# Nathan494326/Husky-Rover-MPPI-IsaacSim

Measured on AMD Instinct MI355X. Metric: MPPI steps/sec at K=65536 H=100 on 750x750 costmap; 1/2/4/8-GPU scaling, higher is better.
Workload: dtype f32

## Files before the change

### husky-rover-mppi-isaacsim_amd/csrc/mppi_kernels.hip

```cpp
#include <hip/hip_runtime.h>

#include <algorithm>
#include <type_traits>
#include <stdint.h>

#include "mppi_detmath.h"
#include "mppi_kernels.h"

namespace mppi {

constexpr bool kFastMath = false;
constexpr bool kChainFast = true;

struct Recip {
  float b, y;
};
__device__ __forceinline__ bool div_ok(float v) {
  const float a = fabsf(v);
  return a >= 9.094947017729282e-13f && a <= 1.099511627776e12f;
}
template <bool F>
__device__ __forceinline__ Recip rc(float b, bool& bad) {
  Recip r;
  r.b = b;
// ... 511 lines not shown
  if (p.mode == 2) return b;
  if (j == 0) return (double)p.m;
  return (double)p.ea * a + (double)p.eb * b;
}
__device__ __forceinline__ PairScale ld_scale(const PairScale* ps) { return *ps; }
__device__ __forceinline__ double pair_apply_raw(const PairScale p, double a, double b, int j) {
  double r = (double)p.ea * a + (double)p.eb * b;
  asm volatile("" : "+v"(r));
  const double n = j == 0 ? (double)p.m : r;
  return p.mode == 1 ? a : (p.mode == 2 ? b : n);
}
__device__ __forceinline__ double pair_apply_sel(const PairScale& ps, double a, double b, int j) {
  return pair_apply_raw(ps, a, b, j);
}

template <int G>
__device__ __forceinline__ void group_scales(const float (&m)[G], float T, PairScale (&ps)[G - 1]) {
  float cur[G];
#pragma unroll
  for (int i = 0; i < G; ++i) cur[i] = m[i];
  int base = 0;
#pragma unroll
  for (int w = G / 2; w >= 1; w >>= 1) {
#pragma unroll
    for (int i = 0; i < w; ++i) {
      ps[base + i] = pair_scale(cur[2 * i], cur[2 * i + 1], T);
      cur[i] = ps[base + i].m;
    }
    base += w;
  }
}
template <int G>
__device__ __forceinline__ double group_apply(const PairScale* ps, const double (&v)[G], int j) {
  double cur[G];
#pragma unroll
  for (int i = 0; i < G; ++i) cur[i] = v[i];
  int base = 0;
#pragma unroll
  for (int w = G / 2; w >= 1; w >>= 1) {
#pragma unroll
    for (int i = 0; i < w; ++i) cur[i] = pair_apply(ps[base + i], cur[2 * i], cur[2 * i + 1], j);
    base += w;
  }
  return cur[0];
}

template <bool FRESH, int NT = 1024>
__device__ __forceinline__ int thread_id() {
  int t = threadIdx.x;
  if constexpr (FRESH) asm volatile("" : "+v"(t));
  __builtin_assume(t >= 0 && t < NT);
  return t;
}

struct NoiseVals {
  float a1, a2, b1, b2;
};
__device__ __forceinline__ NoiseVals noise_gen(uint64_t seed, uint64_t n_base, int64_t k_offset, int blk, int n, int tj) {
  const uint64_t kg = (uint64_t)(k_offset + (int64_t)blk * 256 + tj);
  NoiseVals v;
  noise_block_pk(seed, n_base + (uint64_t)n, kg, &v.a1, &v.a2, &v.b1, &v.b2);
  return v;
}
__device__ __forceinline__ void noise_store(float* __restrict__ eps, int H, int blk, int n, int tj, const NoiseVals& v) {
  const int t = 2 * n;
  float* e1 = eps + ((size_t)blk * 2 * H + t) * 256 + tj;
  float* e2 = e1 + (size_t)H * 256;
  __hip_atomic_store(e1, v.a1, __ATOMIC_RELAXED, __HIP_MEMORY_SCOPE_AGENT);
  __hip_atomic_store(e2, v.a2, __ATOMIC_RELAXED, __HIP_MEMORY_SCOPE_AGENT);
  if (t + 1 < H) {
    __hip_atomic_store(e1 + 256, v.b1, __ATOMIC_RELAXED, __HIP_MEMORY_SCOPE_AGENT);
    __hip_atomic_store(e2 + 256, v.b2, __ATOMIC_RELAXED, __HIP_MEMORY_SCOPE_AGENT);
  }
}
__device__ __forceinline__ void noise_unit(uint64_t seed, uint64_t n_base, int64_t k_offset, int H, int blk, int n,
                                           float* __restrict__ eps, int tj) {
  noise_store(eps, H, blk, n, tj, noise_gen(seed, n_base, k_offset, blk, n, tj));
}
__device__ __forceinline__ void noise_rows(uint64_t seed, uint64_t n_base, int64_t k_offset, int H, int end,
                                           float* __restrict__ eps, int g0, int gstride, int tj) {
  const int NB = (H + 1) >> 1;
  if (g0 >= end) return;
  int blk = g0 / NB, n = g0 - blk * NB;
  const int sq = gstride / NB, sr = gstride - sq * NB;
  for (int g = g0; g < end; g += gstride) {
    noise_unit(seed, n_base, k_offset, H, blk, n, eps, tj);
    blk += sq;
    n += sr;
    if (n >= NB) {
      n -= NB;
      ++blk;
    }
  }
}
struct NoisePos {
  int q, g, blk, n;
};
__device__ __forceinline__ void noise_pos_step(NoisePos& p, int stride, int NB) {
  p.q += stride;
  p.n += (p.q >> 2) - p.g;
  p.g = p.q >> 2;
  while (p.n >= NB) {
    p.n -= NB;
    ++p.blk;
  }
}
// ... 680 lines not shown
      if constexpr (MODE == 0) {
        const int tn = min(p + 2, H - 1);
        e1r = eps_row[(size_t)tn * TB];
        e2r = eps_row[(size_t)(H + tn) * TB];
      }
    };
    using T_ = std::true_type;
    using F_ = std::false_type;
    int p = 0;
    for (const int p1 = min(H, PAIR_LAG) & ~1; p < p1; p += 2) {
      half(F_{}, T_{}, F_{}, p, eA1, eA2, cmA, cmB);
      half(T_{}, T_{}, F_{}, p + 1, eB1, eB2, cmB, cmA);
    }
    if (p == PAIR_LAG) {
      for (; p + 1 < H; p += 2) {
        half(F_{}, T_{}, T_{}, p, eA1, eA2, cmA, cmB);
        half(T_{}, T_{}, T_{}, p + 1, eB1, eB2, cmB, cmA);
      }
    }
    for (; p < H + PAIR_LAG; p += 2) {
      half(F_{}, F_{}, F_{}, p, eA1, eA2, cmA, cmB);
      if (p + 1 < H + PAIR_LAG) half(T_{}, F_{}, F_{}, p + 1, eB1, eB2, cmB, cmA);
    }
    const float cm_last = ((H - 1) & 1) ? cmB : cmA;
    if (cm_last > a.thr) ob = ob + a.pen;
    ob = ob + cm_last;
    float pf;
    if (a.pf_far) {
      const float dx = last_x - a.igx, dy = last_y - a.igy;
      pf = (dx * dx + dy * dy) * a.pf_scale;
    } else {
      pf = pf_sum;
    }
    float cost = a.w_path * pf;
    cost = cost + a.w_slope * sw;
    cost = cost + a.w_speed * sp;
    cost = cost + a.w_obs * ob;
    if (valid) a.cost_out[kl] = cost;
    cost_lds[tj] = valid ? cost : INFINITY;
  }
  __syncthreads();
  if constexpr (MODE == 0)
    leaf_records<TB, NT, true>(a, cost_lds, scratch, a.eps + (size_t)blockIdx.x * (2 * H) * TB, unom_lds, ucache,
                               a.ucache_steps);
  else
    leaf_records<TB, NT>(a, cost_lds, scratch, a.ustore + (size_t)blockIdx.x * (2 * H) * TB);
}

constexpr int kProdPrio = 1, kSidePrio = 0;
constexpr int kProdPrefetch = 2;
constexpr int ROLE_CHAIN = 0, ROLE_PROD = 1, ROLE_WHEEL = 2, ROLE_COST = 3, NROLES = 4;

template <int TB, int PROJ, int MODE, bool DUMP, bool FUSED>
__device__ __forceinline__ int roles_body(const RolloutArgs& a, int blk, unsigned* rec_cnt, int* ticket_lds = nullptr) {
  extern __shared__ __attribute__((aligned(16))) unsigned char smem_raw[];
  constexpr int NT = NROLES * TB;
  constexpr int NG = TB / 64;
  constexpr int D = PAIR_D;
  constexpr int DO = ROLES_RING_OUT;
  constexpr int RI = 4;
  static_assert(TB == 256, "UCACHE_ROW assumes 256 trajectories per workgroup");
  float* ring_in = reinterpret_cast<float*>(smem_raw);
  float* ring_out = ring_in + D * RI * TB;
  float* cost_lds = ring_out + DO * 4 * TB;
  float* sw_lds = cost_lds + TB;
  int* flags = reinterpret_cast<int*>(sw_lds + TB);
  float* unom_lds = reinterpret_cast<float*>(flags + 4 * NG);
  unsigned char* scratch = reinterpret_cast<unsigned char*>(unom_lds + ((2 * a.H + 3) & ~3));
  float* ucache = reinterpret_cast<float*>(
      smem_raw + ((size_t)(scratch - smem_raw) + ((TB + TB / 64) * 4 + 15) / 16 * 16 +
                  (size_t)(TB / 256) * (2 * a.H + 2) * sizeof(double) + 15) / 16 * 16);
  const int tid = thread_id<FUSED, NT>();
  const int wave = __builtin_amdgcn_readfirstlane(tid >> 6);
  const int role = wave / NG;
  const int grp = wave - role * NG;
  const int tj = grp * 64 + (tid & 63);
  if (a.wave_prio) {
    if (role == ROLE_CHAIN) __builtin_amdgcn_s_setprio(3);
    else if (role == ROLE_PROD) __builtin_amdgcn_s_setprio(kProdPrio);
    else __builtin_amdgcn_s_setprio(kSidePrio);
  }
  int* f_prod = flags + grp;
  int* f_chain = flags + NG + grp;
  int* f_wheel = flags + 2 * NG + grp;
  int* f_cost = flags + 3 * NG + grp;
  const int64_t kl = (int64_t)blk * TB + tj;
  const bool valid = kl < a.K;
  const int H = a.H;
  Dem dem;
  dem.init(a.Z, a.rows, a.grid, a.x_min, a.y_min, a.res, a.rinv_res, a.cdiv_res);
  dem.N = a.ntab;
  const float res_half_neg = (-a.res) / 2.0f;
  const float res_sq = a.res * a.res;
  bool nobad = false;
  const bool clk_wg = a.clk != nullptr && blockIdx.x == 0 && tid == 0;
  if (clk_wg) a.clk[4] = __builtin_amdgcn_s_memrealtime();
  const bool clk_any = a.clk != nullptr && tid == 0 && blockIdx.x < kClkBlocks;
  if (clk_any) a.clk[kClkBase + 2 * blockIdx.x] = __builtin_amdgcn_s_memrealtime();
  if (tid < 4 * NG) flags[tid] = 0;
  if constexpr (MODE == 0)
    for (int i = tid; i < 2 * H; i += NT)
      unom_lds[i] = __hip_atomic_load(i < H ? a.u_nom1 + i : a.u_nom2 + (i - H), __ATOMIC_RELAXED,
                                      __HIP_MEMORY_SCOPE_AGENT);
  __syncthreads();

  auto wait_ge = [&](const int* f, int target, int& seen) __attribute__((always_inline)) {
    if (seen >= target) return;
    int v;
    while ((v = lds_load_acquire(f)) < target) __builtin_amdgcn_s_sleep(1);
    seen = v;
  };
  using T_ = std::true_type;
  using F_ = std::false_type;
  float c_pf = 0.f, c_ob = 0.f;

  if (role == ROLE_CHAIN) {
    Traj s;
    s.x = a.x0;
    s.y = a.y0;
    {
      float q[4];
      dem.template corners<false>(s.x, s.y, q, nobad);
      const float vx = res_half_neg * (((q[1] - q[0]) - q[2]) + q[3]);
      const float vy = res_half_neg * (((q[2] - q[0]) - q[1]) + q[3]);
      const float nn = sqrtf((vx * vx + vy * vy) + res_sq * res_sq);
      const float nx = vx / nn, ny = vy / nn, nz = res_sq / nn;
      if constexpr (PROJ == 3) {
        const float d = (a.h0x * nx + a.h0y * ny) + a.h0z * nz;
        const float tx = a.h0x - d * nx, ty = a.h0y - d * ny, tz = a.h0z - d * nz;
        const float tn = sqrtf((tx * tx + ty * ty) + tz * tz);
        s.hx = tx / tn;
        s.hy = ty / tn;
        s.hz = tz / tn;
      } else {
        s.hx = a.h0x;
        s.hy = a.h0y;
        s.hz = a.h0z;
      }
    }
    int seen_prod = 0, seen_wheel = 0, seen_cost = 0;
    if constexpr (PROJ == 3) {
      const int* cons[2] = {f_wheel, f_cost};
      int seen_cons[2] = {0, 0};
      chain_wave_3d<TB, 2, DUMP, DO, !FUSED>(a, dem, s, tj, valid, kl, ring_in, ring_out, f_prod, f_chain, cons,
                                             seen_prod, seen_cons);
    } else
    for (int sc = 0; sc < H; ++sc) {
      wait_ge(f_prod, sc + 1, seen_prod);
      wait_ge(f_wheel, sc - DO + 1, seen_wheel);
      wait_ge(f_cost, sc - DO + 1, seen_cost);
      const float* ri = ring_in + (sc % D) * RI * TB + tj;
      const float v = ri[0], sn = ri[TB], cs = ri[2 * TB];
      const float cx = 0.f, cy = 0.f;
      StepOut o;
      step2d<false>(dem, a.dt, v, sn, cs, s, o, nobad);
      const float z = o.z;
      float* ro = ring_out + (sc % DO) * 4 * TB + tj;
      ro[0] = s.x;
      ro[TB] = s.y;
      ro[2 * TB] = cx;
      ro[3 * TB] = cy;
      if constexpr (DUMP) {
        if (valid) {
          const size_t o3 = ((size_t)kl * H + sc) * 3;
          if (a.d_traj) { a.d_traj[o3] = s.x; a.d_traj[o3 + 1] = s.y; a.d_traj[o3 + 2] = z; }
          if (a.d_hv) { a.d_hv[o3] = s.hx; a.d_hv[o3 + 1] = s.hy; a.d_hv[o3 + 2] = s.hz; }
        }
      }
      lds_store_release(f_chain, sc + 1);
    }
  }
  else if (role == ROLE_PROD) {
    const float* eps_row = (MODE == 0) ? a.eps + (size_t)blk * (2 * H) * TB + tj : nullptr;
    float* ust = a.ustore + (size_t)blk * (2 * H) * TB + tj;
    float L = a.wl, R = a.wr;
    float sp = 0.f;
    int seen_chain = 0;
    constexpr int PF = kProdPrefetch;
    float e[PF][2] = {};
    if constexpr (MODE == 0) {
#pragma unroll
      for (int q = 0; q < PF; ++q) {
        const int t = min(q, H - 1);
        e[q][0] = eps_row[(size_t)t * TB];
        e[q][1] = eps_row[(size_t)(H + t) * TB];
      }
    }
    auto prod = [&](int p, float& e1r, float& e2r) __attribute__((always_inline)) {
      float u1, u2;
      if constexpr (MODE == 0) {
        const int ti = min(p + 1, H - 1);
        u1 = clampf(unom_lds[ti] + a.s1 * e1r, a.min_u1, a.max_u1);
        u2 = clampf(unom_lds[H + ti] + a.s2 * e2r, a.min_u2, a.max_u2);
        if (p < a.ucache_steps) {
          ucache[(size_t)p * UCACHE_ROW + tj] = u1;
          ucache[(size_t)(a.ucache_steps + p) * UCACHE_ROW + tj] = u2;
        }
      } else {
        const size_t o = (size_t)(valid ? kl : 0) * H + p;
        u1 = a.inj_u1[o];
        u2 = a.inj_u2[o];
        ust[(size_t)p * TB] = u1;
        ust[(size_t)(H + p) * TB] = u2;
      }
      L = L * a.fa + (u1 * a.fk) * (1.0f - a.fa);
      R = R * a.fa + (u2 * a.fk) * (1.0f - a.fa);
      const float vp = clampf((L + R) / 2.0f, a.vmin, a.vmax);
      const float wp = clampf(((-L) + R) / a.rwheel, a.wmin, a.wmax);
      float sn, cs;
      if (a.small_angle) dm_sincosf_small(wp * a.dt, &sn, &cs);
      else dm_sincosf(wp * a.dt, &sn, &cs);
      const float spt = sp + (a.vmax - vp) / (vp + 0.0001f);
      sp = a.speed_on ? spt : sp;
      wait_ge(f_chain, p - D + 1, seen_chain);
      float* ri = ring_in + (p % D) * RI * TB + tj;
      ri[0] = vp;
      ri[TB] = sn;
      ri[2 * TB] = cs;
      ri[3 * TB] = 1.0f - cs;
      if constexpr (DUMP) {
        if (valid) {
          const size_t o1 = (size_t)kl * H + p;
          if (a.d_u1) a.d_u1[o1] = u1;
          if (a.d_u2) a.d_u2[o1] = u2;
          if (a.d_w) a.d_w[o1] = wp;
          if (a.d_v) a.d_v[o1] = vp;
        }
      }
      lds_store_release(f_prod, p + 1);
      if constexpr (MODE == 0) {
        const int tn = min(p + PF, H - 1);
        e1r = eps_row[(size_t)tn * TB];
        e2r = eps_row[(size_t)(H + tn) * TB];
      }
    };
    int p = 0;
    for (; p + PF <= H; p += PF) {
#pragma unroll
      for (int q = 0; q < PF; ++q) prod(p + q, e[q][0], e[q][1]);
    }
// ... 20 lines not shown
        ry = y - cy;
        rz = dem.template point<false>(rx, ry, nobad);
      }
      if constexpr (DUMP) {
        if (valid) {
          const size_t o3 = ((size_t)kl * H + sc) * 3;
          if (a.d_lw) { a.d_lw[o3] = lx; a.d_lw[o3 + 1] = ly; a.d_lw[o3 + 2] = lz; }
          if (a.d_rw) { a.d_rw[o3] = rx; a.d_rw[o3 + 1] = ry; a.d_rw[o3 + 2] = rz; }
        }
      }
    };
    auto wstep = [&](auto x_is_a, int sc) __attribute__((always_inline)) {
      constexpr bool XA = decltype(x_is_a)::value;
      float& Xlx = XA ? Alx : Blx; float& Xly = XA ? Aly : Bly; float& Xlz = XA ? Alz : Blz;
      float& Xrx = XA ? Arx : Brx; float& Xry = XA ? Ary : Bry; float& Xrz = XA ? Arz : Brz;
      const float& Ylx = XA ? Blx : Alx; const float& Yly = XA ? Bly : Aly; const float& Ylz = XA ? Blz : Alz;
      const float& Yrx = XA ? Brx : Arx; const float& Yry = XA ? Bry : Ary; const float& Yrz = XA ? Brz : Arz;
      const int i = sc - 4;
      if (i >= 0 && i < H - 3) {
        const float term = slope_term<false>(Xlx, Xly, Xlz, Ylx, Yly, Ylz, Xrx, Xry, Xrz, Yrx, Yry, Yrz, nobad);
        sw = sw + term;
      }
      contacts(sc, Xlx, Xly, Xlz, Xrx, Xry, Xrz);
      if constexpr (DUMP) {
        if (sc + 1 < H) {
          float lx, ly, lz, rx, ry, rz;
          contacts(sc + 1, lx, ly, lz, rx, ry, rz);
        }
        lds_store_release(f_wheel, min(sc + 2, H));
      } else {
        lds_store_release(f_wheel, min(sc + 2, H));
      }
    };
    int sc = 0;
    for (; sc + 2 < H; sc += 4) {
      wstep(T_{}, sc);
      wstep(F_{}, sc + 2);
    }
    if (sc < H) {
      wstep(T_{}, sc);
      sc += 2;
    }
    const int last = sc - 2;
    const int i = last - 2;
    if (i >= 0 && i < H - 3) {
      const float term = (last % 4 == 0)
          ? slope_term<false>(Blx, Bly, Blz, Alx, Aly, Alz, Brx, Bry, Brz, Arx, Ary, Arz, nobad)
          : slope_term<false>(Alx, Aly, Alz, Blx, Bly, Blz, Arx, Ary, Arz, Brx, Bry, Brz, nobad);
      sw = sw + term;
    }
    sw_lds[tj] = sw;
  } else {
    int seen_chain = 0;
    float pf_sum = 0.f, ob = 0.f, last_x = a.x0, last_y = a.y0;
    float cmA = 0.f, cmB = 0.f;
    Recip rcm;
    rcm.b = a.res_c;
    auto cstep = [&](int sc, float& cm_mine, float& cm_prev) __attribute__((always_inline)) {
      wait_ge(f_chain, sc + 1, seen_chain);
      const float* ro = ring_out + (sc % DO) * 4 * TB + tj;
      const float x = ro[0], y = ro[TB];
      cm_mine = a.cm[costmap_index<false>(a.cm_size, a.hw, rcm, x, y, nobad, a.rinv_res_c, a.cdiv_res_c)];
      const float pft = pf_sum + 10.0f * (fabsf(x - a.gx) + fabsf(y - a.gy));
      pf_sum = (sc < H - 1) ? pft : pf_sum;
      last_x = x;
      last_y = y;
      const float ob1 = (cm_prev > a.thr) ? ob + a.pen : ob;
      ob = (sc > 0) ? ob1 + cm_prev : ob;
      if constexpr (DUMP) {
      }
      lds_store_release(f_cost, sc + 1);
    };
    int sc = 0;
    for (; sc + 1 < H; sc += 2) {
      cstep(sc, cmA, cmB);
      cstep(sc + 1, cmB, cmA);
    }
    if (sc < H) cstep(sc, cmA, cmB);
    const float cm_last = ((H - 1) & 1) ? cmB : cmA;
    if (cm_last > a.thr) ob = ob + a.pen;
    ob = ob + cm_last;
    float pf;
    if (a.pf_far) {
      const float dx = last_x - a.igx, dy = last_y - a.igy;
      pf = (dx * dx + dy * dy) * a.pf_scale;
    } else {
      pf = pf_sum;
    }
    c_pf = pf;
    c_ob = ob;
  }
  __syncthreads();
  if (clk_wg) a.clk[5] = __builtin_amdgcn_s_memrealtime();
  if (role == ROLE_COST) {
    float cost = a.w_path * c_pf;
    cost = cost + a.w_slope * sw_lds[tj];
    cost = cost + a.w_speed * cost_lds[tj];
    cost = cost + a.w_obs * c_ob;
    if (valid) a.cost_out[kl] = cost;
    cost_lds[tj] = valid ? cost : INFINITY;
  }
  __syncthreads();
  if constexpr (MODE == 0)
    leaf_records<TB, NT, true, FUSED>(a, cost_lds, scratch, a.eps + (size_t)blk * (2 * H) * TB, unom_lds,
                                      ucache, a.ucache_steps, blk);
  else
// ... 637 lines not shown
    }
    v0 = v[0];
#pragma unroll
    for (int q = 0; q < 6; ++q)
      if ((1 << q) < NGW) sh[q] = ld_scale(lps + colfin_level_base(P, 4 + q) + (it_g >> (q + 1)));
  }
  int lvl = 4;
#pragma unroll
  for (int q = 0; q < 6; ++q) {
    const int k = 1 << q;
    if (k < NGW) {
      const double o = __shfl_xor(v0, k, 64);
      if (has_item && (it_g & (2 * k - 1)) == 0) v0 = pair_apply_raw(sh[q], v0, o, col);
      ++lvl;
    }
  }
  if (has_item && (it_g & (NGW - 1)) == 0) part[it_c * NG + it_g] = v0;
  __syncthreads();
  for (int stride = NGW; stride < NG; stride *= 2, ++lvl) {
    const int w = NG / (2 * stride);
    const PairScale* ps = lps + colfin_level_base(P, lvl);
    for (int it = tid; it < ncols * w; it += FIN_THREADS) {
      const int c = it % ncols, i = it / ncols;
      const int cc = (c < nc) ? c0 + c : 1;
      double* pc = part + c * NG;
      pc[2 * stride * i] = pair_apply_sel(ps[i], pc[2 * stride * i], pc[2 * stride * i + stride], cc);
    }
    __syncthreads();
  }
  if (f.mode == 0) {
    for (int c = tid; c < nc; c += FIN_THREADS) f.record_out[c0 + c] = part[c * NG];
    return true;
  }
  const double S = extra_s ? part[nc * NG] : part[(1 - c0) * NG];
  float ures = 0.0f;
  if (nblk == 1) {
    if (tid < 2 * H) ures = (S > 0.0) ? (float)(part[(tid + 2) * NG] / S) : 0.0f;
    __syncthreads();
    if (RECS_WT && tid == 0) __hip_atomic_store(rec_cnt, 0u, __ATOMIC_RELAXED, __HIP_MEMORY_SCOPE_AGENT);
  } else {
    const unsigned long long tag = (unsigned long long)f.seq << 32;
    for (int c = tid; c < nc; c += FIN_THREADS) {
      const int j = c0 + c;
      if (j >= 2) {
        const float u = (S > 0.0) ? (float)(part[c * NG] / S) : 0.0f;
        __hip_atomic_store(f.uopt + (j - 2), tag | __builtin_bit_cast(unsigned, u), __ATOMIC_RELAXED,
                           __HIP_MEMORY_SCOPE_AGENT);
      }
    }
    if (blk != nblk - 1) return true;
    int late = 0;
    if (tid < 2 * H) {
      const uint64_t t0 = __builtin_amdgcn_s_memrealtime();
      unsigned long long w = __hip_atomic_load(f.uopt + tid, __ATOMIC_RELAXED, __HIP_MEMORY_SCOPE_AGENT);
      while ((unsigned)(w >> 32) != f.seq) {
        if (__builtin_amdgcn_s_memrealtime() - t0 >= kColfinPollTicks ||
            (f.abort && __hip_atomic_load(f.abort, __ATOMIC_RELAXED, __HIP_MEMORY_SCOPE_AGENT) == f.seq)) {
          late = 1;
          break;
        }
        __builtin_amdgcn_s_sleep(1);
        w = __hip_atomic_load(f.uopt + tid, __ATOMIC_RELAXED, __HIP_MEMORY_SCOPE_AGENT);
      }
      ures = __builtin_bit_cast(float, (unsigned)w);
    }
    if (__syncthreads_or(late)) return false;
    if (RECS_WT && tid == 0) __hip_atomic_store(rec_cnt, 0u, __ATOMIC_RELAXED, __HIP_MEMORY_SCOPE_AGENT);
  }
  __syncthreads();
  finish_phase2(f, ures, smem_raw, tid, FIN_THREADS, qpre);
  return true;
}

__global__ __launch_bounds__(FIN_THREADS) void mppi_colfin_kernel(const FinishArgs f, int P, int ncol) {
  (void)colfin_body<false>(f, P, ncol, (int)blockIdx.x, (int)gridDim.x, nullptr);
}

__global__ __launch_bounds__(TAIL_THREADS) void mppi_tail_kernel(const FinishArgs f) {
  extern __shared__ __attribute__((aligned(16))) unsigned char smem_raw[];
  const int tid = threadIdx.x;
  const int H = f.H;
  float4* in4 = reinterpret_cast<float4*>(smem_raw);
  float* chain = reinterpret_cast<float*>(in4 + H + 1);
  if (tid == 0 && f.clk) f.clk[kClkServer + 8 * (f.seq & 7) + 4] = __builtin_amdgcn_s_memrealtime();
  auto ld = [&](int i) { return __hip_atomic_load(f.tail_in + i, __ATOMIC_RELAXED, __HIP_MEMORY_SCOPE_AGENT); };
  for (int t = tid; t <= H; t += TAIL_THREADS) {
    if (t == H) {
      in4[H] = make_float4(ld(0), 0.f, 0.f, 0.f);
    } else {
      const float cs = ld(2 * H + t);
      in4[t] = make_float4(ld(min(t + 1, H - 1)), ld(H + t), cs, 1.0f - cs);
    }
  }
  __syncthreads();
  Dem dem;
  dem.init(f.Z, f.rows, f.grid, f.x_min, f.y_min, f.res, f.rinv_res, f.cdiv_res);
  dem.N = f.ntab;
  optimal_rollout(f, dem, in4, chain, H, f.tail_out, tid, TAIL_THREADS);
  if (tid == 0 && f.clk) f.clk[kClkServer + 8 * (f.seq & 7) + 5] = __builtin_amdgcn_s_memrealtime();
}

__global__ __launch_bounds__(256) void mppi_bilinear_kernel(const float* __restrict__ Z, int rows,
                                                            int grid, float x_min, float y_min,
                                                            float res, const float* __restrict__ xs,
                                                            const float* __restrict__ ys,
                                                            float* __restrict__ hs, int64_t n) {
  Dem dem;
  dem.init(Z, rows, grid, x_min, y_min, res);
  const int64_t stride = (int64_t)gridDim.x * blockDim.x;
  for (int64_t i = (int64_t)blockIdx.x * blockDim.x + threadIdx.x; i < n; i += stride) {
    const float x = xs[i], y = ys[i];
    float q[4];
    bool bad = false;
    dem.template corners<true>(x, y, q, bad);
    float h = bilinear<true>(x, y, q, dem.template rr<true>(), bad);
    if (bad) {
      dem.template corners<false>(x, y, q, bad);
// ... 556 lines not shown

__global__ __launch_bounds__(256) void mppi_normal_table_kernel(const float* __restrict__ Z, int rows, int grid,
                                                                float res, float4* __restrict__ out) {
  const int64_t cols = (int64_t)grid + 1;
  const int64_t n = ((int64_t)rows + 1) * cols;
  const float res_half_neg = (-res) / 2.0f;
  const float res_sq = res * res;
  for (int64_t g = (int64_t)blockIdx.x * 256 + threadIdx.x; g < n; g += (int64_t)gridDim.x * 256) {
    const int j = (int)(g / cols) - 1, i = (int)(g % cols) - 1;
    const int r0 = clampi(j, 0, rows - 1), r1 = clampi(j + 1, 0, rows - 1);
    const int c0 = clampi(i, 0, grid - 1), c1 = clampi(i + 1, 0, grid - 1);
    const float q0 = Z[(size_t)r0 * grid + c0], q1 = Z[(size_t)r0 * grid + c1];
    const float q2 = Z[(size_t)r1 * grid + c0], q3 = Z[(size_t)r1 * grid + c1];
    bool unused = false;
    const float vx = res_half_neg * (((q1 - q0) - q2) + q3);
    const float vy = res_half_neg * (((q2 - q0) - q1) + q3);
    const Recip r = rc<false>(sq<false>((vx * vx + vy * vy) + res_sq * res_sq, unused), unused);
    out[g] = make_float4(dv<false>(vx, r, unused), dv<false>(vy, r, unused), dv<false>(res_sq, r, unused), 0.0f);
  }
}

hipError_t launch_normal_table(const float* Z, int rows, int grid, float res, float4* out, hipStream_t st) {
  const int64_t n = ((int64_t)rows + 1) * ((int64_t)grid + 1);
  const unsigned blocks = (unsigned)std::min<int64_t>((n + 255) / 256, 256 * 16);
  hipLaunchKernelGGL(mppi_normal_table_kernel, dim3(blocks), dim3(256), 0, st, Z, rows, grid, res, out);
  return hipGetLastError();
}

__global__ __launch_bounds__(256) void mppi_noise_kernel(uint64_t seed, uint64_t n_base, int64_t k_offset,
                                                         int H, int n_blocks, float* __restrict__ eps) {
  noise_rows(seed, n_base, k_offset, H, n_blocks * ((H + 1) >> 1), eps, blockIdx.x, gridDim.x, threadIdx.x);
}

struct ServerLaunch {
  RolloutArgs a;
  ServerArgs z;
};
__device__ __forceinline__ const ServerLaunch* fresh_args() {
#if __HIP_DEVICE_COMPILE__
  uint64_t v = reinterpret_cast<uint64_t>(__builtin_amdgcn_kernarg_segment_ptr());
  asm volatile("" : "+s"(v));
  return (const ServerLaunch*)reinterpret_cast<const __attribute__((address_space(4))) ServerLaunch*>(v);
#else
  return nullptr;
#endif
}

template <int TB, int PROJ>
__global__ __launch_bounds__(NROLES * TB) __attribute__((amdgpu_num_vgpr(56))) void mppi_step_server_kernel(
    const ServerLaunch args) {
  __shared__ unsigned cmd_lds[32];
  __shared__ int sh[2];
  const int tid = threadIdx.x;
  unsigned expect = args.z.first_seq;
  bool head = blockIdx.x == 0;
  for (;;) {
    const auto* L = fresh_args();
    const ServerArgs& z = L->z;
    if (tid < 64) {
      const int slot = tid < kCmdWords ? tid : 0;
      const unsigned long long* src =
          (head ? reinterpret_cast<const unsigned long long*>(z.cmd->slot) : z.relay) + slot;
      const unsigned* host_stop = reinterpret_cast<const unsigned*>(z.cmd->slot + kCmdStopSlot);
      unsigned ok = 0;
      unsigned long long w = 0;
      const uint64_t t0 = __builtin_amdgcn_s_memrealtime();
      uint64_t t_stop = t0;
      if (tid == 0 && head && z.clk) z.clk[kClkServer + 8 * (expect & 7) + 6] = t0;
      const bool forced = head && z.exit_after != 0 && expect - z.first_seq >= z.exit_after;
      while (!forced) {
        w = head ? __hip_atomic_load(src, __ATOMIC_RELAXED, __HIP_MEMORY_SCOPE_SYSTEM)
                 : __hip_atomic_load(src, __ATOMIC_RELAXED, __HIP_MEMORY_SCOPE_AGENT);
        const unsigned lo = (unsigned)w, hi = (unsigned)(w >> 32);
        const unsigned long long stop_slot = (unsigned)__builtin_amdgcn_readlane((int)lo, kCmdStopSlot);
        if (cmd_stop_hit(stop_slot, z.launch_id)) break;
        const unsigned seq0 = (unsigned)__builtin_amdgcn_readfirstlane((int)hi);
        if (__builtin_amdgcn_ballot_w64(!cmd_slot_ok(slot, w, seq0, expect)) == 0) {
          ok = 1;
          break;
        }
        const uint64_t now = __builtin_amdgcn_s_memrealtime();
        if (head) {
          if (now - t0 >= z.idle_ticks) break;
        } else {
          if (now - t_stop >= 10000) {
            t_stop = now;
            if (__hip_atomic_load(host_stop, __ATOMIC_RELAXED, __HIP_MEMORY_SCOPE_SYSTEM) == z.launch_id) break;
          }
          __builtin_amdgcn_s_sleep(2);
        }
      }
      if (ok && tid < kCmdWords) {
        if (head && tid != kCmdStopSlot)
          __hip_atomic_store(z.relay + tid, w, __ATOMIC_RELAXED, __HIP_MEMORY_SCOPE_AGENT);
        cmd_lds[tid] = (unsigned)w;
      }
      if (head && !ok && tid == 0)
        __hip_atomic_store(z.relay + kCmdStopSlot, (unsigned long long)z.launch_id, __ATOMIC_RELAXED,
                           __HIP_MEMORY_SCOPE_AGENT);
      if (tid == 0) cmd_lds[31] = ok;
      if (tid == 0 && head && z.clk && ok)
        __hip_atomic_store(z.clk + kClkServer + 8 * (cmd_lds[0] & 7), (uint64_t)__builtin_amdgcn_s_memrealtime(),
                           __ATOMIC_RELAXED, __HIP_MEMORY_SCOPE_AGENT);
    }
    __syncthreads();
    if (!cmd_lds[31]) return;
    const ServerCmd& c = *reinterpret_cast<const ServerCmd*>(cmd_lds);
    auto rd = [&](const float& x) __attribute__((always_inline)) {
      return __builtin_bit_cast(float, __builtin_amdgcn_readfirstlane(__builtin_bit_cast(int, x)));
    };
    const unsigned seq = __builtin_amdgcn_readfirstlane(c.seq);
    const int eps_slot = __builtin_amdgcn_readfirstlane(c.eps_slot);
    const int cur = __builtin_amdgcn_readfirstlane(c.cur);
    RolloutArgs a = L->a;
    a.eps = z.eps[eps_slot];
    a.u_nom1 = z.u_nom[cur];
    a.u_nom2 = z.u_nom[cur] + a.H;
    a.x0 = rd(c.x0);
    a.y0 = rd(c.y0);
    a.h0x = rd(c.h0x);
    a.h0y = rd(c.h0y);
    a.h0z = rd(c.h0z);
    a.wl = rd(c.wl);
    a.wr = rd(c.wr);
    a.gx = rd(c.gx);
    a.gy = rd(c.gy);
    a.s1 = rd(c.s1);
    a.s2 = rd(c.s2);
    a.igx = rd(c.igx);
    a.igy = rd(c.igy);
    a.pf_scale = rd(c.pf_scale);
    a.pf_far = __builtin_amdgcn_readfirstlane(c.pf_far);
    a.speed_on = __builtin_amdgcn_readfirstlane(c.speed_on);
    const int nslot = __builtin_amdgcn_readfirstlane(c.noise_slot);
    const uint64_t nbase = ((uint64_t)__builtin_amdgcn_readfirstlane(c.noise_n_base_hi) << 32) |
                           (uint32_t)__builtin_amdgcn_readfirstlane(c.noise_n_base_lo);
    const int64_t W = 4 * (int64_t)z.nroll * ((a.H + 1) >> 1);
    const int nn = z.nroll - z.fin_groups;
    const int64_t S = 2 * (int64_t)nn + z.fin_groups - 1;
    const int ticket = roles_body<TB, PROJ, 0, false, true>(a, (int)blockIdx.x, z.rec_cnt, sh);
    if (ticket == z.nroll - 1 && tid == 0 && z.clk) {
      const uint64_t now = __builtin_amdgcn_s_memrealtime();
      z.clk[kClkServer + 8 * (seq & 7) + 1] = now;
      const uint64_t t0 = __hip_atomic_load(z.clk + kClkServer + 8 * (seq & 7), __ATOMIC_RELAXED, __HIP_MEMORY_SCOPE_AGENT);
      __hip_atomic_fetch_add(z.clk + kClkSums, now - t0, __ATOMIC_RELAXED, __HIP_MEMORY_SCOPE_AGENT);
      __hip_atomic_fetch_add(z.clk + kClkSums + 1, (uint64_t)1, __ATOMIC_RELAXED, __HIP_MEMORY_SCOPE_AGENT);
    }
    const int blk = ticket - (z.nroll - z.fin_groups);
    if (blk < 0 && nslot >= 0) {
      __builtin_amdgcn_s_setprio(0);
      const int wave = __builtin_amdgcn_readfirstlane(tid >> 6);
      const int q0 = (int)(W * (2 * ticket) / S), q1 = (int)(W * (2 * ticket + 2) / S);
      noise_waves(a.seed, nbase, a.k_offset, a.H, q0 + wave, q1, NROLES * TB / 64, z.eps[nslot], tid & 63);
    }
    if (blk >= 0) {
      __builtin_amdgcn_s_setprio(0);
      if (tid == 0) {
        const uint64_t t0 = __builtin_amdgcn_s_memrealtime();
        int late = z.wait_ticks == 0;
        while (!late && ticket != z.nroll - 1 &&
               __hip_atomic_load(z.rec_cnt, __ATOMIC_RELAXED, __HIP_MEMORY_SCOPE_AGENT) < (unsigned)z.nroll) {
          if (__builtin_amdgcn_s_memrealtime() - t0 >= z.wait_ticks ||
              __hip_atomic_load(z.f.abort, __ATOMIC_RELAXED, __HIP_MEMORY_SCOPE_AGENT) == seq) {
            late = 1;
            break;
          }
          __builtin_amdgcn_s_sleep(2);
        }
        if (late) __hip_atomic_store(z.f.abort, seq, __ATOMIC_RELAXED, __HIP_MEMORY_SCOPE_AGENT);
        sh[1] = late;
      }
      __syncthreads();
      bool ok = !sh[1];
      if (ok) {
        FinishArgs f = z.f;
        const int mode = __builtin_amdgcn_readfirstlane(c.mode);
        const int slot = __builtin_amdgcn_readfirstlane(c.tail_slot);
        f.mode = mode;
        f.seq = seq;
        f.u_nom_next = z.u_nom[cur ^ 1];
        f.tail_in = z.tail_in[slot];
        f.tail_out = z.tail_out[slot];
        f.x0 = a.x0;
        f.y0 = a.y0;
        f.h0x = a.h0x;
        f.h0y = a.h0y;
        f.h0z = a.h0z;
        f.wl = a.wl;
        f.wr = a.wr;
        ok = colfin_body<true>(f, z.fin_P, z.fin_ncol, blk, z.fin_groups, z.rec_cnt);
        if (ok && blk == z.fin_groups - 1 && tid == 0 && z.clk) {
          const uint64_t now = __builtin_amdgcn_s_memrealtime();
          z.clk[kClkServer + 8 * (seq & 7) + 2] = now;
          const uint64_t t0 = __hip_atomic_load(z.clk + kClkServer + 8 * (seq & 7), __ATOMIC_RELAXED, __HIP_MEMORY_SCOPE_AGENT);
          __hip_atomic_fetch_add(z.clk + kClkSums + 2, now - t0, __ATOMIC_RELAXED, __HIP_MEMORY_SCOPE_AGENT);
          __hip_atomic_fetch_add(z.clk + kClkSums + 3, (uint64_t)1, __ATOMIC_RELAXED, __HIP_MEMORY_SCOPE_AGENT);
        }
      }
      if (!ok && tid == 0)
        __hip_atomic_store(z.f.done, seq | kDoneFail, __ATOMIC_RELAXED, __HIP_MEMORY_SCOPE_SYSTEM);
      if (nslot >= 0 && blk < z.fin_groups - 1) {
        const int wave = __builtin_amdgcn_readfirstlane(tid >> 6);
        const int q0 = (int)(W * (2 * nn + blk) / S), q1 = (int)(W * (2 * nn + blk + 1) / S);
        noise_waves(a.seed, nbase, a.k_offset, a.H, q0 + wave, q1, NROLES * TB / 64, z.eps[nslot], tid & 63);
      }
    }
    if (tid == 0) __builtin_amdgcn_fence(__ATOMIC_ACQUIRE, "agent");
    expect = seq + 1;
    head = ticket == z.nroll - 1;
    __syncthreads();
    if (tid == 0 && z.clk) {
      const uint64_t now = __builtin_amdgcn_s_memrealtime();
      if (blk < 0) __hip_atomic_fetch_max(z.clk + kClkServer + 8 * (seq & 7) + 3, now, __ATOMIC_RELAXED, __HIP_MEMORY_SCOPE_AGENT);
      __hip_atomic_fetch_max(z.clk + kClkServer + 8 * (seq & 7) + 7, now, __ATOMIC_RELAXED, __HIP_MEMORY_SCOPE_AGENT);
    }
  }
}

hipError_t launch_step_server(const RolloutArgs& a, const ServerArgs& z, size_t lds, hipStream_t st, int proj) {
  const dim3 g((unsigned)z.nroll), b(NROLES * 256);
  if (proj == 3)
    hipLaunchKernelGGL((mppi_step_server_kernel<256, 3>), g, b, lds, st, ServerLaunch{a, z});
  else
    hipLaunchKernelGGL((mppi_step_server_kernel<256, 2>), g, b, lds, st, ServerLaunch{a, z});
  return hipGetLastError();
}

hipError_t launch_noise(uint64_t seed, uint64_t n_base, int64_t k_offset, int blocks, int H, float* eps,
                        hipStream_t st, int max_groups) {
  const int NB = (H + 1) >> 1;
  const int64_t total = (int64_t)blocks * NB;
  const unsigned grid = (unsigned)std::min<int64_t>(total, std::max(max_groups, 1));
  hipLaunchKernelGGL(mppi_noise_kernel, dim3(grid), dim3(256), 0, st, seed, n_base, k_offset, H, blocks, eps);
  return hipGetLastError();
}

__global__ __launch_bounds__(256) void mppi_cdiv_verify_kernel(float b, float y, unsigned* bad) {
  const unsigned i = blockIdx.x * 256u + threadIdx.x;
  const float a = __builtin_bit_cast(float, 0x3f800000u | i);
  const float q = cdiv_f(a, b, y);
  const float ref = a / b;
  if (__builtin_bit_cast(unsigned, q) != __builtin_bit_cast(unsigned, ref)) atomicAdd(bad, 1u);
}

__global__ __launch_bounds__(64) void mppi_hold_kernel(uint64_t ticks) {
  extern __shared__ unsigned char hold_lds[];
  const uint64_t t0 = __builtin_amdgcn_s_memrealtime();
  hold_lds[threadIdx.x] = 0;
  while (__builtin_amdgcn_s_memrealtime() - t0 < ticks) __builtin_amdgcn_s_sleep(64);
}

hipError_t launch_hold(int groups, size_t lds, uint64_t ticks, hipStream_t st) {
  hipLaunchKernelGGL(mppi_hold_kernel, dim3((unsigned)groups), dim3(64), lds, st, ticks);
  return hipGetLastError();
}

hipError_t launch_cdiv_verify(float b, float y, unsigned* bad, hipStream_t st) {
  hipLaunchKernelGGL(mppi_cdiv_verify_kernel, dim3(1u << 15), dim3(256), 0, st, b, y, bad);
  return hipGetLastError();
}
// ... 21 lines not shown
```

Baseline: 13270.

## Pipeline head command polling with multiple in-flight loads and hoist first loads

Replaces the persistent server's command polling loop with a poll helper that keeps several loads in flight. The head block uses hand-written inline assembly that issues four outstanding system-scope loads, cutting latency when a new command arrives. Polling moves from wave 0 to the first cost-role wave, and leftover in-flight loads are drained after the chain role publishes its first step. The chain's first DEM corner fetch and the producer's eps prefetch are also hoisted before the role split so they overlap. The inline asm with manual vmcnt handling is fragile, and the extra outstanding loads add memory traffic.

```diff
diff --git a/husky-rover-mppi-isaacsim_amd/csrc/mppi_kernels.hip b/husky-rover-mppi-isaacsim_amd/csrc/mppi_kernels.hip
--- a/husky-rover-mppi-isaacsim_amd/csrc/mppi_kernels.hip
+++ b/husky-rover-mppi-isaacsim_amd/csrc/mppi_kernels.hip
@@ -587,6 +587,102 @@
   __builtin_assume(t >= 0 && t < NT);
   return t;
 }
+
+template <int N, typename V, typename Ld, typename Hit, typename Quit>
+__device__ __forceinline__ int poll_in_flight(V& out, Ld ld, Hit hit, Quit quit) {
+  V r[N];
+#pragma unroll
+  for (int k = 0; k < N; ++k) r[k] = ld();
+  for (;;) {
+#pragma unroll
+    for (int k = 0; k < N; ++k) {
+      const int verdict = hit(r[k]);
+      if (verdict || quit(r[k])) {
+        out = r[k];
+        return verdict;
+      }
+      r[k] = ld();
+    }
+  }
+}
+constexpr int kHeadPollDepth = 4, kFinPollDepth = 1;
+static_assert(kHeadPollDepth == 1 || kHeadPollDepth == 4, "the head's poll is written for 1 or 4 reads in flight");
+
+struct HeadSweeps {
+  unsigned long long r0 = 0, r1 = 0, r2 = 0, r3 = 0;
+  int phase = 4;
+  __device__ __forceinline__ bool resume(const unsigned long long* src, unsigned long long ref, uint64_t deadline,
+                                         unsigned long long& cand) {
+    int st;
+    uint64_t now;
+#if __HIP_DEVICE_COMPILE__
+    asm volatile(
+        "s_cmp_eq_u32 %[ph], 4\n"
+        "s_cbranch_scc0 1f\n"
+        "global_load_dwordx2 %[r0], %[src], off sc0 sc1\n"
+        "global_load_dwordx2 %[r1], %[src], off sc0 sc1\n"
+        "global_load_dwordx2 %[r2], %[src], off sc0 sc1\n"
+        "global_load_dwordx2 %[r3], %[src], off sc0 sc1\n"
+        "s_waitcnt vmcnt(3)\n"
+        "s_branch 10f\n"
+        "1:\n"
+        "s_cmp_eq_u32 %[ph], 1\n"
+        "s_cbranch_scc1 21f\n"
+        "s_cmp_eq_u32 %[ph], 2\n"
+        "s_cbranch_scc1 22f\n"
+        "s_cmp_eq_u32 %[ph], 3\n"
+        "s_cbranch_scc1 23f\n"
+#define MPPI_HEAD_SLOT(L, R, HIT)                                                    \
+        L ":\n"                                                                      \
+        "s_waitcnt vmcnt(3)\n"                                                       \
+        "v_cmp_ne_u64 vcc, " R ", %[ref]\n"                                         \
+        "s_cmp_lg_u64 vcc, 0\n"                                                      \
+        "s_cbranch_scc1 " HIT "f\n"                                                  \
+        "s_memrealtime %[now]\n"                                                     \
+        "s_waitcnt lgkmcnt(0)\n"                                                     \
+        "v_cmp_gt_u64 vcc, %[now], %[dl]\n"                                          \
+        "s_cmp_lg_u64 vcc, 0\n"                                                      \
+        "s_cbranch_scc1 90f\n"                                                       \
+        "global_load_dwordx2 " R ", %[src], off sc0 sc1\n"
+        MPPI_HEAD_SLOT("20", "%[r0]", "10")
+        MPPI_HEAD_SLOT("21", "%[r1]", "11")
+        MPPI_HEAD_SLOT("22", "%[r2]", "12")
+        MPPI_HEAD_SLOT("23", "%[r3]", "13")
+#undef MPPI_HEAD_SLOT
+        "s_branch 20b\n"
+#define MPPI_HEAD_HIT(L, R, NEXT)                                                    \
+        L ":\n"                                                                      \
+        "v_mov_b64 %[cand], " R "\n"                                                \
+        "global_load_dwordx2 " R ", %[src], off sc0 sc1\n"                          \
+        "s_mov_b32 %[ph], " NEXT "\n"                                               \
+        "s_mov_b32 %[st], 1\n"                                                       \
+        "s_branch 99f\n"
+        MPPI_HEAD_HIT("10", "%[r0]", "1")
+        MPPI_HEAD_HIT("11", "%[r1]", "2")
+        MPPI_HEAD_HIT("12", "%[r2]", "3")
+        MPPI_HEAD_HIT("13", "%[r3]", "0")
+#undef MPPI_HEAD_HIT
+        "90:\n"
+        "s_mov_b32 %[st], 0\n"
+        "99:\n"
+        : [r0] "+v"(r0), [r1] "+v"(r1), [r2] "+v"(r2), [r3] "+v"(r3), [ph] "+s"(phase), [cand] "=&v"(cand),
+          [st] "=&s"(st), [now] "=&s"(now)
+        : [src] "v"(src), [ref] "v"(ref), [dl] "v"(deadline)
+        : "vcc", "scc", "memory");
+#else
+    st = 0;
+    now = 0;
+#endif
+    (void)now;
+    return st != 0;
+  }
+  __device__ __forceinline__ void drain() {
+#if __HIP_DEVICE_COMPILE__
+    asm volatile("s_waitcnt vmcnt(0)  ; sweeps in %0 %1 %2 %3" : "+v"(r0), "+v"(r1), "+v"(r2), "+v"(r3)::"memory");
+#endif
+    phase = 4;
+  }
+};
 
 struct NoiseVals {
   float a1, a2, b1, b2;
@@ -1373,7 +1469,8 @@
 constexpr int ROLE_CHAIN = 0, ROLE_PROD = 1, ROLE_WHEEL = 2, ROLE_COST = 3, NROLES = 4;
 
 template <int TB, int PROJ, int MODE, bool DUMP, bool FUSED>
-__device__ __forceinline__ int roles_body(const RolloutArgs& a, int blk, unsigned* rec_cnt, int* ticket_lds = nullptr) {
+__device__ __forceinline__ int roles_body(const RolloutArgs& a, int blk, unsigned* rec_cnt, int* ticket_lds = nullptr,
+                                          HeadSweeps* pend = nullptr) {
   extern __shared__ __attribute__((aligned(16))) unsigned char smem_raw[];
   constexpr int NT = NROLES * TB;
   constexpr int NG = TB / 64;
@@ -1424,6 +1521,22 @@
       unom_lds[i] = __hip_atomic_load(i < H ? a.u_nom1 + i : a.u_nom2 + (i - H), __ATOMIC_RELAXED,
                                       __HIP_MEMORY_SCOPE_AGENT);
   __syncthreads();
+  constexpr int PF = kProdPrefetch;
+  const float* eps_row = (MODE == 0) ? a.eps + (size_t)blk * (2 * H) * TB + tj : nullptr;
+  float q_first[4] = {0.f, 0.f, 0.f, 0.f};
+  float e[PF][2] = {};
+  if (role == ROLE_CHAIN) {
+    dem.template corners<false>(a.x0, a.y0, q_first, nobad);
+  } else if (role == ROLE_PROD) {
+    if constexpr (MODE == 0) {
+#pragma unroll
+      for (int q = 0; q < PF; ++q) {
+        const int t = min(q, H - 1);
+        e[q][0] = eps_row[(size_t)t * TB];
+        e[q][1] = eps_row[(size_t)(H + t) * TB];
+      }
+    }
+  }
 
   auto wait_ge = [&](const int* f, int target, int& seen) __attribute__((always_inline)) {
     if (seen >= target) return;
@@ -1440,8 +1553,7 @@
     s.x = a.x0;
     s.y = a.y0;
     {
-      float q[4];
-      dem.template corners<false>(s.x, s.y, q, nobad);
+      const float (&q)[4] = q_first;
       const float vx = res_half_neg * (((q[1] - q[0]) - q[2]) + q[3]);
       const float vy = res_half_neg * (((q[2] - q[0]) - q[1]) + q[3]);
       const float nn = sqrtf((vx * vx + vy * vy) + res_sq * res_sq);
@@ -1492,21 +1604,10 @@
     }
   }
   else if (role == ROLE_PROD) {
-    const float* eps_row = (MODE == 0) ? a.eps + (size_t)blk * (2 * H) * TB + tj : nullptr;
     float* ust = a.ustore + (size_t)blk * (2 * H) * TB + tj;
     float L = a.wl, R = a.wr;
     float sp = 0.f;
     int seen_chain = 0;
-    constexpr int PF = kProdPrefetch;
-    float e[PF][2] = {};
-    if constexpr (MODE == 0) {
-#pragma unroll
-      for (int q = 0; q < PF; ++q) {
-        const int t = min(q, H - 1);
-        e[q][0] = eps_row[(size_t)t * TB];
-        e[q][1] = eps_row[(size_t)(H + t) * TB];
-      }
-    }
     auto prod = [&](int p, float& e1r, float& e2r) __attribute__((always_inline)) {
       float u1, u2;
       if constexpr (MODE == 0) {
@@ -1633,6 +1734,12 @@
     sw_lds[tj] = sw;
   } else {
     int seen_chain = 0;
+    if constexpr (FUSED) {
+      if (pend != nullptr && grp == 0) {
+        wait_ge(f_chain, 1, seen_chain);
+        pend->drain();
+      }
+    }
     float pf_sum = 0.f, ob = 0.f, last_x = a.x0, last_y = a.y0;
     float cmA = 0.f, cmB = 0.f;
     Recip rcm;
@@ -2376,17 +2483,26 @@
     int late = 0;
     if (tid < 2 * H) {
       const uint64_t t0 = __builtin_amdgcn_s_memrealtime();
-      unsigned long long w = __hip_atomic_load(f.uopt + tid, __ATOMIC_RELAXED, __HIP_MEMORY_SCOPE_AGENT);
-      while ((unsigned)(w >> 32) != f.seq) {
-        if (__builtin_amdgcn_s_memrealtime() - t0 >= kColfinPollTicks ||
-            (f.abort && __hip_atomic_load(f.abort, __ATOMIC_RELAXED, __HIP_MEMORY_SCOPE_AGENT) == f.seq)) {
-          late = 1;
-          break;
-        }
-        __builtin_amdgcn_s_sleep(1);
-        w = __hip_atomic_load(f.uopt + tid, __ATOMIC_RELAXED, __HIP_MEMORY_SCOPE_AGENT);
-      }
-      ures = __builtin_bit_cast(float, (unsigned)w);
+      struct WordAbort {
+        unsigned long long w;
+        unsigned abort;
+      } wa;
+      const unsigned no_abort = ~f.seq;
+      late = !poll_in_flight<kFinPollDepth>(
+          wa,
+          [&]() {
+            WordAbort v;
+            v.w = __hip_atomic_load(f.uopt + tid, __ATOMIC_RELAXED, __HIP_MEMORY_SCOPE_AGENT);
+            v.abort = f.abort ? __hip_atomic_load(f.abort, __ATOMIC_RELAXED, __HIP_MEMORY_SCOPE_AGENT) : no_abort;
+            return v;
+          },
+          [&](const WordAbort& v) { return (unsigned)(v.w >> 32) == f.seq ? 1 : 0; },
+          [&](const WordAbort& v) {
+            if (__builtin_amdgcn_s_memrealtime() - t0 >= kColfinPollTicks || v.abort == f.seq) return true;
+            __builtin_amdgcn_s_sleep(1);
+            return false;
+          });
+      ures = __builtin_bit_cast(float, (unsigned)wa.w);
     }
     if (__syncthreads_or(late)) return false;
     if (RECS_WT && tid == 0) __hip_atomic_store(rec_cnt, 0u, __ATOMIC_RELAXED, __HIP_MEMORY_SCOPE_AGENT);
@@ -3049,13 +3165,16 @@
   __shared__ unsigned cmd_lds[32];
   __shared__ int sh[2];
   const int tid = threadIdx.x;
+  constexpr int kPollTid0 = ROLE_COST * TB;
   unsigned expect = args.z.first_seq;
   bool head = blockIdx.x == 0;
   for (;;) {
     const auto* L = fresh_args();
     const ServerArgs& z = L->z;
-    if (tid < 64) {
-      const int slot = tid < kCmdWords ? tid : 0;
+    const int plane = thread_id<true, NROLES * TB>() - kPollTid0;
+    HeadSweeps pend;
+    if (plane >= 0 && plane < 64) {
+      const int slot = plane < kCmdWords ? plane : 0;
       const unsigned long long* src =
           (head ? reinterpret_cast<const unsigned long long*>(z.cmd->slot) : z.relay) + slot;
       const unsigned* host_stop = reinterpret_cast<const unsigned*>(z.cmd->slot + kCmdStopSlot);
@@ -3063,40 +3182,59 @@
       unsigned long long w = 0;
       const uint64_t t0 = __builtin_amdgcn_s_memrealtime();
       uint64_t t_stop = t0;
-      if (tid == 0 && head && z.clk) z.clk[kClkServer + 8 * (expect & 7) + 6] = t0;
+      if (plane == 0 && head && z.clk) z.clk[kClkServer + 8 * (expect & 7) + 6] = t0;
       const bool forced = head && z.exit_after != 0 && expect - z.first_seq >= z.exit_after;
-      while (!forced) {
-        w = head ? __hip_atomic_load(src, __ATOMIC_RELAXED, __HIP_MEMORY_SCOPE_SYSTEM)
-                 : __hip_atomic_load(src, __ATOMIC_RELAXED, __HIP_MEMORY_SCOPE_AGENT);
-        const unsigned lo = (unsigned)w, hi = (unsigned)(w >> 32);
+      auto sweep = [&](unsigned long long v) __attribute__((always_inline)) {
+        const unsigned lo = (unsigned)v, hi = (unsigned)(v >> 32);
         const unsigned long long stop_slot = (unsigned)__builtin_amdgcn_readlane((int)lo, kCmdStopSlot);
-        if (cmd_stop_hit(stop_slot, z.launch_id)) break;
+        if (cmd_stop_hit(stop_slot, z.launch_id)) return 2;
         const unsigned seq0 = (unsigned)__builtin_amdgcn_readfirstlane((int)hi);
-        if (__builtin_amdgcn_ballot_w64(!cmd_slot_ok(slot, w, seq0, expect)) == 0) {
-          ok = 1;
-          break;
+        return __builtin_amdgcn_ballot_w64(!cmd_slot_ok(slot, v, seq0, expect)) == 0 ? 1 : 0;
+      };
+      if (head) {
+        if (!forced) {
+          if constexpr (kHeadPollDepth == 1) {
+            ok = poll_in_flight<1>(
+                     w, [&]() { return __hip_atomic_load(src, __ATOMIC_RELAXED, __HIP_MEMORY_SCOPE_SYSTEM); }, sweep,
+                     [&](unsigned long long) { return __builtin_amdgcn_s_memrealtime() - t0 >= z.idle_ticks; }) == 1;
+          } else {
+            const uint64_t deadline = t0 + z.idle_ticks;
+            unsigned long long ref = 0;
+            while (pend.resume(src, ref, deadline, w)) {
+              const int verdict = sweep(w);
+              if (verdict) {
+                ok = verdict == 1;
+                break;
+              }
+              ref = w;
+            }
+            if (!ok) pend.drain();
+          }
         }
-        const uint64_t now = __builtin_amdgcn_s_memrealtime();
-        if (head) {
-          if (now - t0 >= z.idle_ticks) break;
-        } else {
-          if (now - t_stop >= 10000) {
-            t_stop = now;
-            if (__hip_atomic_load(host_stop, __ATOMIC_RELAXED, __HIP_MEMORY_SCOPE_SYSTEM) == z.launch_id) break;
-          }
-          __builtin_amdgcn_s_sleep(2);
-        }
-      }
-      if (ok && tid < kCmdWords) {
-        if (head && tid != kCmdStopSlot)
-          __hip_atomic_store(z.relay + tid, w, __ATOMIC_RELAXED, __HIP_MEMORY_SCOPE_AGENT);
-        cmd_lds[tid] = (unsigned)w;
-      }
-      if (head && !ok && tid == 0)
+      } else {
+        ok = poll_in_flight<1>(
+                 w, [&]() { return __hip_atomic_load(src, __ATOMIC_RELAXED, __HIP_MEMORY_SCOPE_AGENT); }, sweep,
+                 [&](unsigned long long) {
+                   const uint64_t now = __builtin_amdgcn_s_memrealtime();
+                   if (now - t_stop >= 10000) {
+                     t_stop = now;
+                     if (__hip_atomic_load(host_stop, __ATOMIC_RELAXED, __HIP_MEMORY_SCOPE_SYSTEM) == z.launch_id)
+                       return true;
+                   }
+                   __builtin_amdgcn_s_sleep(2);
+                   return false;
+                 }) == 1;
+      }
+      if (ok && plane < kCmdWords) {
+        if (head && plane != kCmdStopSlot)
+          __hip_atomic_store(z.relay + plane, w, __ATOMIC_RELAXED, __HIP_MEMORY_SCOPE_AGENT);
+        cmd_lds[plane] = (unsigned)w;
+      }
+      if (head && !ok && plane == 0)
         __hip_atomic_store(z.relay + kCmdStopSlot, (unsigned long long)z.launch_id, __ATOMIC_RELAXED,
                            __HIP_MEMORY_SCOPE_AGENT);
-      if (tid == 0) cmd_lds[31] = ok;
-      if (tid == 0 && head && z.clk && ok)
+      if (plane == 0) cmd_lds[31] = ok;
+      if (plane == 0 && head && z.clk && ok)
         __hip_atomic_store(z.clk + kClkServer + 8 * (cmd_lds[0] & 7), (uint64_t)__builtin_amdgcn_s_memrealtime(),
                            __ATOMIC_RELAXED, __HIP_MEMORY_SCOPE_AGENT);
     }
@@ -3135,7 +3273,7 @@
     const int64_t W = 4 * (int64_t)z.nroll * ((a.H + 1) >> 1);
     const int nn = z.nroll - z.fin_groups;
     const int64_t S = 2 * (int64_t)nn + z.fin_groups - 1;
-    const int ticket = roles_body<TB, PROJ, 0, false, true>(a, (int)blockIdx.x, z.rec_cnt, sh);
+    const int ticket = roles_body<TB, PROJ, 0, false, true>(a, (int)blockIdx.x, z.rec_cnt, sh, &pend);
     if (ticket == z.nroll - 1 && tid == 0 && z.clk) {
       const uint64_t now = __builtin_amdgcn_s_memrealtime();
       z.clk[kClkServer + 8 * (seq & 7) + 1] = now;
@@ -3155,14 +3293,20 @@
       if (tid == 0) {
         const uint64_t t0 = __builtin_amdgcn_s_memrealtime();
         int late = z.wait_ticks == 0;
-        while (!late && ticket != z.nroll - 1 &&
-               __hip_atomic_load(z.rec_cnt, __ATOMIC_RELAXED, __HIP_MEMORY_SCOPE_AGENT) < (unsigned)z.nroll) {
-          if (__builtin_amdgcn_s_memrealtime() - t0 >= z.wait_ticks ||
-              __hip_atomic_load(z.f.abort, __ATOMIC_RELAXED, __HIP_MEMORY_SCOPE_AGENT) == seq) {
-            late = 1;
-            break;
-          }
-          __builtin_amdgcn_s_sleep(2);
+        if (!late && ticket != z.nroll - 1) {
+          uint2 ca;
+          late = !poll_in_flight<kFinPollDepth>(
+              ca,
+              [&]() {
+                return make_uint2(__hip_atomic_load(z.rec_cnt, __ATOMIC_RELAXED, __HIP_MEMORY_SCOPE_AGENT),
+                                  __hip_atomic_load(z.f.abort, __ATOMIC_RELAXED, __HIP_MEMORY_SCOPE_AGENT));
+              },
+              [&](uint2 v) { return v.x >= (unsigned)z.nroll ? 1 : 0; },
+              [&](uint2 v) {
+                if (__builtin_amdgcn_s_memrealtime() - t0 >= z.wait_ticks || v.y == seq) return true;
+                __builtin_amdgcn_s_sleep(2);
+                return false;
+              });
         }
         if (late) __hip_atomic_store(z.f.abort, seq, __ATOMIC_RELAXED, __HIP_MEMORY_SCOPE_AGENT);
         sh[1] = late;
@@ -3202,7 +3346,7 @@
         noise_waves(a.seed, nbase, a.k_offset, a.H, q0 + wave, q1, NROLES * TB / 64, z.eps[nslot], tid & 63);
       }
     }
-    if (tid == 0) __builtin_amdgcn_fence(__ATOMIC_ACQUIRE, "agent");
+    if (thread_id<true, NROLES * TB>() == kPollTid0) __builtin_amdgcn_fence(__ATOMIC_ACQUIRE, "agent");
     expect = seq + 1;
     head = ticket == z.nroll - 1;
     __syncthreads();
```

After: 13230. Within noise of the previous version (-0.3%).
